# mayataka/robotoc

Hardware: NVIDIA H100
Metric: SQP-iterations/s (ANYmal N=40, batch=1024) at 1/2/4/8 H100 vs CPU ref (higher is better)
Workload: dtype f64

## Files before the change

### robotoc_b200/csrc/rbt_api.cu

```cuda
#include <cmath>
#include <cstdio>
#include <cstring>
#include <cstdint>
#include <cstdlib>
#include <string>
#include <utility>
#include <vector>

#include <cuda_runtime.h>
#include <dlfcn.h>

#include <algorithm>

#include "../../include/robotoc_b200.h"
#include "riccati_backward.cuh"
#include "riccati_forward.cuh"
#include "riccati_time_parallel.cuh"
#include "riccati_unconstr.cuh"
#include "stage_kernels.cuh"
#include "ustage_kernels.cuh"
#include "eval_kernels.cuh"
#include "line_search_kernels.cuh"
#include "rnea_kernels.cuh"
#include "contact_kernels.cuh"
// ... 88 lines not shown
  long long per;
  int scope;
  bool stage;
  Bindable* bind;
  int in;
};

long long buf_doubles(const BufDesc& d, bool stage_ready, int batch, int n_grid) {
  if (d.scope == SC_NONE || (d.stage && !stage_ready)) return -1;
  return d.per * batch * (d.scope == SC_GRID ? n_grid : 1);
}

struct Win {
  int b0, nb, n_grid;
  size_t rec() const { return size_t(b0) * n_grid; }
};

long long plan_bytes(const std::vector<Copy>& plan, bool up) {
  long long bytes = 0;
  for (const Copy& c : plan)
    if (c.up == up) bytes += (long long)(c.width * 8 * c.rows);
  return bytes;
}

}

struct rbt_handle {
  rbt_dims dims;
  rbt_layout L;
  int n_grid_max = 0, n_grid = 0, batch = 0, device = 0;
  double max_dts0 = 0.1;
  DevBuf<rbt_stage_ctrl> d_ctrl;
  std::vector<rbt_stage_ctrl> ctrl;
  Bindable d_kkt, d_ric, d_fact, d_dir, d_dx0;
  DevBuf<int> d_info;
  DevBuf<int> d_struct;
  int fxx_mode = RBT_FXX_AUTO;
  int tsegs = 0, n_sm = 0;
  DevBuf<double> d_tp_elem, d_tp_scan[2], d_tp_fmap, d_tp_dx;
  DevBuf<int> d_tp_fail;
  const double* tp_seeds = nullptr;
  bool kkt_from_condense = false;
  bool stage_ready = false;
  bool keep_info = false;
  rbt_stage_dims sdims;
  rbt_stage_layout S;
  rbt_constraint_table table;
  Bindable d_lin, d_con, d_ex, d_sol, d_xd;
  DevBuf<double> d_steps, d_ones;
  DevBuf<double> d_stage_perf, d_perf, d_x0in;
  DevBuf<int> d_tgt;
  DevBuf<double> d_limits;
  DevBuf<rbt::RneaModel> d_model;
  DevBuf<double> d_gains;
  DevBuf<double> d_cpos;
  bool cpos_set = false;
  int ls_trials = 0;
  DevBuf<double> d_ls_alphas, d_ls_trial, d_ls_stage_barrier, d_ls_barrier, d_ls_in, d_ls_filt, d_ls_step;
  DevBuf<int> d_ls_nfilt, d_ls_k;
  DevBuf<double> d_step_pack;
  long long launches = 0;
  DevBuf<double> d_wire;
  DevBuf<double> d_res_stage;
  DevBuf<double> d_sd_stage;
  DevBuf<rbt_wire_layout> d_W;
  long long w_ocp = 0;
// ... 37 lines not shown
  rbt_ulayout L;
  rbt_make_ulayout(nv, &L);
  return rbt_ulayout_field(&L, field);
}

int rbt_device_info(int device, int* sm, int* n_sm, char* name, int name_len) {
  cudaDeviceProp prop;
  if (cudaGetDeviceProperties(&prop, device) != cudaSuccess) {
    cudaGetLastError();
    return RBT_ERR_CUDA;
  }
  if (sm) *sm = prop.major * 10 + prop.minor;
  if (n_sm) *n_sm = prop.multiProcessorCount;
  if (name && name_len > 0) {
    std::strncpy(name, prop.name, name_len - 1);
    name[name_len - 1] = 0;
  }
  return RBT_OK;
}

int rbt_create(const rbt_dims* dims, int n_grid_max, int batch, int device, rbt_handle** out) {
  if (!dims || !out || n_grid_max < 2 || batch < 1 || dims->nv < 1 || dims->nu < 1 || dims->ns_max < 0) return RBT_ERR_ARG;
  if (dims->nv != CNV || dims->nu != CNU || dims->ns_max != CNS) return RBT_ERR_ARG;
  rbt_handle* h = new rbt_handle();
  h->dims = *dims;
  rbt_make_layout(dims, &h->L);
  h->n_grid_max = n_grid_max;
  h->batch = batch;
  h->device = device;
  *out = h;
  RBT_CUDA(h, cudaSetDevice(device));
  const size_t per = size_t(batch) * n_grid_max;
  RBT_CUDA(h, h->d_ctrl.ensure(size_t(n_grid_max)));
  RBT_CUDA(h, zeroed(h->d_kkt.own, per * h->L.k_stride));
  RBT_CUDA(h, zeroed(h->d_ric.own, per * h->L.r_stride));
  RBT_CUDA(h, zeroed(h->d_fact.own, per * h->L.f_stride));
  RBT_CUDA(h, zeroed(h->d_dir.own, per * h->L.d_stride));
  RBT_CUDA(h, h->d_dx0.own.ensure(size_t(batch) * h->L.nx));
  RBT_CUDA(h, zeroed(h->d_info, size_t(batch)));
  RBT_CUDA(h, zeroed(h->d_struct, 4));
  RBT_CUDA(h, cudaDeviceGetAttribute(&h->n_sm, cudaDevAttrMultiProcessorCount, device));
  return RBT_OK;
}

static int check_contacts(rbt_handle* h, const rbt_stage_dims& sd, const rbt_stage_ctrl* ctrl, int n_grid) {
  for (int i = 0; i < n_grid; ++i)
    if (ctrl[i].nf > sd.nf_max || ctrl[i].contact_mask >= (1 << sd.n_contacts)) {
      h->err = "[rbt_set_schedule] invalid argument: grid " + std::to_string(i) + " has more contacts than the stage layer was set up for";
      return RBT_ERR_ARG;
    }
  return RBT_OK;
}

int rbt_destroy(rbt_handle* h) {
  if (!h) return RBT_ERR_ARG;
  cudaSetDevice(h->device);
  delete h;
  return RBT_OK;
}

int rbt_set_schedule(rbt_handle* h, const rbt_stage_ctrl* ctrl, int n_grid, double max_dts0) {
  if (!h || !ctrl) return RBT_ERR_ARG;
  if (n_grid < 2 || n_grid > h->n_grid_max) {
    h->err = "[rbt_set_schedule] invalid argument: n_grid must be in [2, n_grid_max]";
    return RBT_ERR_ARG;
  }
  if (!(max_dts0 > 0)) {
    h->err = "[rbt_set_schedule] invalid argument: max_dts0 must be positive";
    return RBT_ERR_ARG;
  }
  for (int i = 0; i < n_grid; ++i) {
    const rbt_stage_ctrl& c = ctrl[i];
    const bool last = (i == n_grid - 1);
    if ((c.type == RBT_TERMINAL) != last || c.type < 0 || c.type > 3 || c.ns < 0 || c.ns > h->dims.ns_max ||
        (c.type == RBT_IMPACT && (i == 0 || last)) || (c.type == RBT_LIFT && i == 0)) {
      h->err = "[rbt_set_schedule] invalid argument: inconsistent stage control table at grid " + std::to_string(i);
      return RBT_ERR_ARG;
    }
    const int nf_max = 3 * RBT_MAX_CONTACTS;
    if (c.nf < 0 || c.nf > nf_max || c.nf % 3 != 0 || c.contact_mask < 0 || c.contact_mask >= (1 << RBT_MAX_CONTACTS) ||
        3 * __builtin_popcount((unsigned)c.contact_mask) != c.nf || c.ngrids_in_phase < 0 || !(c.dt >= 0.0) ||
        !(c.dt < 1.0e300) || (c.sto != 0 && c.sto != 1) || (c.sto_next != 0 && c.sto_next != 1) || c.ineq_gate < 0 ||
        c.ineq_gate > 2) {
      h->err = "[rbt_set_schedule] invalid argument: grid " + std::to_string(i) +
               ": need 0 <= nf <= 12, nf % 3 == 0, 3 * popcount(contact_mask) == nf, ngrids_in_phase >= 0, finite dt >= 0, "
               "ineq_gate in {0, 1, 2}";
      return RBT_ERR_ARG;
    }
    if (c.type == RBT_IMPACT && c.ns != 0) {
      h->err = "[rbt_set_schedule] invalid argument: an impact grid carries no switching constraint (grid " + std::to_string(i) + ")";
      return RBT_ERR_ARG;
    }
  }
  if (h->stage_ready && check_contacts(h, h->sdims, ctrl, n_grid) != RBT_OK) return RBT_ERR_ARG;
  RBT_CUDA(h, cudaSetDevice(h->device));
  RBT_CUDA(h, cudaMemcpy(h->d_ctrl.get(), ctrl, sizeof(rbt_stage_ctrl) * n_grid, cudaMemcpyHostToDevice));
  RBT_CUDA(h, cudaMemset(h->d_ric.get(), 0, size_t(h->batch) * n_grid * h->L.r_stride * 8));
  RBT_CUDA(h, cudaMemset(h->d_dir.get(), 0, size_t(h->batch) * n_grid * h->L.d_stride * 8));
  h->n_grid = n_grid;
  h->max_dts0 = max_dts0;
  h->ctrl.assign(ctrl, ctrl + n_grid);
  h->wire_dirty = true;
  return RBT_OK;
}

static BufDesc buf(rbt_handle* h, int which) {
  const rbt_layout& L = h->L;
  const rbt_stage_layout& S = h->S;
  const BufDesc t[] = {
       {h->d_kkt.get(), L.k_stride, SC_GRID, false, &h->d_kkt, IN_KKT},
       {h->d_ric.get(), L.r_stride, SC_GRID, false, &h->d_ric, -1},
       {h->d_fact.get(), L.f_stride, SC_GRID, false, &h->d_fact, -1},
       {h->d_dir.get(), L.d_stride, SC_GRID, false, &h->d_dir, -1},
       {h->d_dx0.get(), L.nx, SC_OCP, false, &h->d_dx0, IN_DX0},
       {nullptr, 0, SC_NONE, false, nullptr, -1},
       {h->d_lin.get(), S.l_stride, SC_GRID, true, &h->d_lin, IN_LIN},
       {h->d_con.get(), S.c_stride, SC_GRID, true, &h->d_con, IN_CON},
       {h->d_ex.get(), S.e_stride, SC_GRID, true, &h->d_ex, -1},
       {h->d_sol.get(), S.s_stride, SC_GRID, true, &h->d_sol, IN_SOL},
       {h->d_xd.get(), S.x_stride, SC_GRID, true, &h->d_xd, -1},
       {h->d_steps.get(), 2, SC_OCP, true, nullptr, -1},
       {h->d_perf.get(), 8, SC_OCP, true, nullptr, -1},
       {h->d_cpos.get(), 3 * S.ncon, SC_GRID, true, nullptr, IN_CPOS},
  };
  return which >= 0 && which < int(sizeof(t) / sizeof(t[0])) ? t[which] : BufDesc{nullptr, 0, SC_NONE, false, nullptr, -1};
}

long long rbt_buf_doubles(rbt_handle* h, int which) {
  return h ? buf_doubles(buf(h, which), h->stage_ready, h->batch, h->n_grid) : -1;
// ... 526 lines not shown
  rbt::StageParams p;
  const rbt_stage_layout& S = h->S;
  const size_t g0 = w.rec();
  p.K = h->L;
  p.S = S;
  p.tab = h->table;
  p.ctrl = h->d_ctrl.get();
  p.n_grid = h->n_grid;
  p.batch = w.nb;
  p.lin = h->d_lin.get() + g0 * S.l_stride;
  p.con = h->d_con.get() + g0 * S.c_stride;
  p.kkt = h->d_kkt.get() + g0 * h->L.k_stride;
  p.ex = h->d_ex.get() + g0 * S.e_stride;
  p.dir = h->d_dir.get() + g0 * h->L.d_stride;
  p.xd = h->d_xd.get() + g0 * S.x_stride;
  p.sol = h->d_sol.get() + g0 * S.s_stride;
  p.steps = h->d_steps.get() + 2 * size_t(w.b0);
  p.info = h->d_info.get() + w.b0;
  p.tgt = reinterpret_cast<const int4*>(h->d_tgt.get());
  p.row_level = h->d_tgt.get() + RBT_MAX_TARGETS * 4;
  return p;
}

#define RBT_STAGE_CHECK(h, what)                                  \
  if (!(h)) return RBT_ERR_ARG;                                   \
  if (!(h)->stage_ready || (h)->n_grid == 0) {                    \
    (h)->err = "[" what "] stage layer not set up / no schedule"; \
    return RBT_ERR_STATE;                                         \
  }                                                               \
  RBT_CUDA(h, cudaSetDevice((h)->device));

static int condense(rbt_handle* h, Win w, cudaStream_t st) {
  using C = rbt::CondCfg<CNV, CNU, CNS>;
  auto kern = rbt::condense_kernel<CNV, CNU, CNS>;
  if (!h->attr_cond) {
    RBT_CUDA(h, cudaFuncSetAttribute(kern, cudaFuncAttributeMaxDynamicSharedMemorySize, (int)C::SMEM_BYTES));
    h->attr_cond = true;
  }
  RBT_CUDA(h, cudaMemsetAsync(h->d_info.get() + w.b0, 0, size_t(w.nb) * sizeof(int), st));
  rbt::mjtjinv_kernel<CNV, CNU><<<(w.nb * h->n_grid + 1) / 2, 64, 0, st>>>(make_stage_params(h, w));
  RBT_CUDA(h, cudaGetLastError());
  if (h->ev_condense_mid) RBT_CUDA(h, cudaEventRecord(h->ev_condense_mid, st));
  kern<<<w.nb * h->n_grid, C::NTHREADS, C::SMEM_BYTES, st>>>(make_stage_params(h, w));
  RBT_CUDA(h, cudaGetLastError());
  h->launches += 2;
  h->keep_info = true;
  h->kkt_from_condense = true;
  return RBT_OK;
}

int rbt_condense(rbt_handle* h, void* stream) {
  RBT_STAGE_CHECK(h, "rbt_condense");
  return condense(h, full(h), (cudaStream_t)stream);
}

int rbt_set_condense_event(rbt_handle* h, void* cuda_event) {
  if (!h) return RBT_ERR_ARG;
  h->ev_condense_mid = (cudaEvent_t)cuda_event;
  return RBT_OK;
}

static int expand(rbt_handle* h, Win w, cudaStream_t st) {
  RBT_CUDA(h, cudaMemcpyAsync(h->d_steps.get() + 2 * size_t(w.b0), h->d_ones.get(), size_t(w.nb) * 2 * 8, cudaMemcpyDeviceToDevice, st));
  rbt::expand_kernel<CNV, CNU, CNS><<<w.nb * h->n_grid, rbt::XTHR, 0, st>>>(make_stage_params(h, w));
  RBT_CUDA(h, cudaGetLastError());
  h->launches += 1;
  return RBT_OK;
}

int rbt_expand_and_step_sizes(rbt_handle* h, void* stream) {
  RBT_STAGE_CHECK(h, "rbt_expand_and_step_sizes");
  return expand(h, full(h), (cudaStream_t)stream);
}

static int update(rbt_handle* h, Win w, cudaStream_t st) {
  rbt::update_kernel<CNV, CNU, CNS><<<w.nb * h->n_grid, rbt::XTHR, 0, st>>>(make_stage_params(h, w));
  RBT_CUDA(h, cudaGetLastError());
  h->launches += 1;
// ... 822 lines not shown
```

### robotoc_b200/csrc/stage_kernels.cuh

```cuda
#pragma once
#include "rbt_device.cuh"
#include "riccati_backward.cuh"
#include "../../include/rbt_stage_layout.h"

namespace rbt {

#define RBT_MAX_TARGETS 96
struct StageParams {
  rbt_layout K;
  rbt_stage_layout S;
  rbt_constraint_table tab;
  const rbt_stage_ctrl* ctrl;
  int n_grid;
  int batch;
  const double* lin;
  double* con;
  double* kkt;
  double* ex;
  double* dir;
  double* xd;
  double* sol;
  double* steps;
  int* info;
  const int4* tgt;
  const int* row_level;
};

__device__ __forceinline__ void cta_gemm(int ta, int tb, int m, int n, int k, double alpha, const double* A, int lda,
                                         const double* B, int ldb, double beta, double* C, int ldc) {
  for (int e = threadIdx.x; e < m * n; e += blockDim.x) {
    const int i = e % m, j = e / m;
    double acc = 0.0;
    for (int l = 0; l < k; ++l) {
      const double a = ta ? A[l + i * lda] : A[i + l * lda];
      const double b = tb ? B[j + l * ldb] : B[l + j * ldb];
      acc = fma(a, b, acc);
    }
    const double c0 = (beta == 0.0) ? 0.0 : beta * C[i + j * ldc];
    C[i + j * ldc] = fma(alpha, acc, c0);
  }
}

__device__ __forceinline__ void inv3_dev(const double* A, int lda, double* B, int ldb) {
  const double a = A[0], b = A[lda], c = A[2 * lda], d = A[1], e = A[1 + lda], f = A[1 + 2 * lda], g = A[2], h = A[2 + lda],
               i = A[2 + 2 * lda];
  const double det = a * (e * i - f * h) - b * (d * i - f * g) + c * (d * h - e * g);
  const double r = 1.0 / det;
  B[0] = (e * i - f * h) * r; B[ldb] = (c * h - b * i) * r; B[2 * ldb] = (b * f - c * e) * r;
  B[1] = (f * g - d * i) * r; B[1 + ldb] = (a * i - c * g) * r; B[1 + 2 * ldb] = (c * d - a * f) * r;
  B[2] = (d * h - e * g) * r; B[2 + ldb] = (b * g - a * h) * r; B[2 + 2 * ldb] = (a * e - b * d) * r;
}

__device__ __noinline__ void se3_jac_inverse_dev(const double* Jac, double* Jinv) {
  double tmp[9];
  for (int q = 0; q < 36; ++q) Jinv[q] = 0.0;
  inv3_dev(Jac, 6, Jinv, 6);
  inv3_dev(Jac + 3 + 18, 6, Jinv + 3 + 18, 6);
  for (int j = 0; j < 3; ++j)
// ... 194 lines not shown
template <int NV, int NU, int NFM>
struct CondCfg {
  static constexpr int NX = 2 * NV, NVF = NV + NFM;
  static constexpr int TX = num_tiles(NX), TF = num_tiles(NVF), TV = num_tiles(NV), TU = num_tiles(NU), TM = num_tiles(NFM);
  static constexpr int NWARPS = TX;
  static constexpr int NTHREADS = 32 * NWARPS;
  static constexpr int up2(int x) { return (x + 1) & ~1; }
  static constexpr int i_D = 0, i_IDC = i_D + up2(NVF * NX), i_Qaa = i_IDC + up2(NVF), i_Qff = i_Qaa + up2(NV),
                       i_Qqf = i_Qff + up2(NFM * NFM), IN1A = i_Qqf + up2(NV * NFM);
  static constexpr int i_Quu = IN1A, i_lx = i_Quu + up2(NU * NU), i_la = i_lx + up2(NX), i_lf = i_la + up2(NV),
                       i_lu = i_lf + up2(NFM), i_Fx = i_lu + up2(NU), i_lup = i_Fx + up2(NX), i_se3 = i_lup + 6,
                       IN1 = i_se3 + 108, IN1B = IN1 - IN1A;
  static constexpr int j_ha = 0, j_hf = j_ha + up2(NV), j_hx = j_hf + up2(NFM), j_hu = j_hx + up2(NX), j_fx = j_hu + up2(NU),
                       j_sc = j_fx + up2(NX), IN2 = j_sc + 4;
  static constexpr int o_in1 = 0;
  static constexpr int o_Z = o_in1 + IN1;
  static constexpr int o_R = o_Z + NVF * NVF;
  static constexpr int o_in2 = o_R + NVF * NX;
  static constexpr int o_vec = o_in2 + IN2;
  static constexpr int v_r = 0, v_laf = NVF, v_haf = 2 * NVF, v_Fi = 3 * NVF, v_FiS = v_Fi + 36, v_dQq = v_FiS + 36,
                       v_dQv = v_dQq + NV * NV, v_end = v_dQv + up2(NV);
  static constexpr int o_bar = (o_vec + v_end + 1) & ~1;
  static constexpr int SMEM_DOUBLES = o_bar + 2;
  static constexpr size_t SMEM_BYTES = size_t(SMEM_DOUBLES) * 8;
  static constexpr int QAF = 0, QUF = NFM * NX;
  static_assert(TF < NWARPS && TV <= NWARPS && 2 * TM < NWARPS, "one warp per row band, one warp left for the vectors");
  static_assert(NFM * NX + NFM * NV <= NVF * NX, "Qaf | Quf fit in the dIDCdqv buffer");
  static_assert((NFM * NX) % 2 == 0 && (NFM * NV) % 2 == 0, "Qaf | Quf are adjacent in the expansion record (one bulk store)");
};

#ifndef RBT_COND_MIN_CTAS
#define RBT_COND_MIN_CTAS 5
#endif
template <int NV, int NU, int NFM>
__global__ void __launch_bounds__(CondCfg<NV, NU, NFM>::NTHREADS, RBT_COND_MIN_CTAS) condense_kernel(const StageParams p) {
  using C = CondCfg<NV, NU, NFM>;
  constexpr int NX = C::NX, NVF = C::NVF, NTHR = C::NTHREADS, TX = C::TX, TF = C::TF, TV = C::TV, TU = C::TU, TM = C::TM;
  extern __shared__ __align__(16) double smem[];
  const rbt_layout& K = p.K;
  const rbt_stage_layout& S = p.S;
  const int tid = threadIdx.x, warp = tid >> 5, lane = tid & 31, g = lane >> 2, t = lane & 3;
  const size_t o = blockIdx.x;
  if (o >= size_t(p.batch) * p.n_grid) return;
  const int i = int(o % p.n_grid);
  const rbt_stage_ctrl c = p.ctrl[i];
  const double* lin = p.lin + o * S.l_stride;
  double* con = p.con + o * S.c_stride;
  double* kkt = p.kkt + o * K.k_stride;
  double* ex = p.ex + o * S.e_stride;
  constexpr int np = NV - NU;

  if (c.type == RBT_TERMINAL) {
    for (int e = tid; e < NX * NX; e += NTHR) kkt[K.k_Qxx + e] = lin[S.l_Qxx + e];
    for (int e = tid; e < NX; e += NTHR) kkt[K.k_lx + e] = lin[S.l_lx + e];
    if (np == 6 && tid == 0) se3_jac_inverse_dev(lin + S.l_se3 + 36, ex + S.e_Fqqpi);
    return;
  }
  const bool impact = (c.type == RBT_IMPACT);
  const bool pdipm = !impact || p.tab.impact_friction_cone != 0;
  const int nf = c.nf, nvf = NV + nf, ns = impact ? 0 : c.ns;
  const double dt = c.dt;
  double* in1 = smem + C::o_in1;
  double* sD = in1 + C::i_D;
  double* sQaf = sD + C::QAF;
  double* sQuf = sD + C::QUF;
  double* vIDC = in1 + C::i_IDC;
  double* vQaa = in1 + C::i_Qaa;
  double* sQff = in1 + C::i_Qff;
  double* sQqf = in1 + C::i_Qqf;
  const double* gQxx = lin + S.l_Qxx;
  double* gQuu = in1 + C::i_Quu;
  double* vlx = in1 + C::i_lx;
  double* vla = in1 + C::i_la;
  double* vlf = in1 + C::i_lf;
  double* vlu = in1 + C::i_lu;
  double* vFx = in1 + C::i_Fx;
  const double* vlup = in1 + C::i_lup;
  const double* sse3 = in1 + C::i_se3;
  double* sZ = smem + C::o_Z;
  double* sR = smem + C::o_R;
  const double* in2 = smem + C::o_in2;
  const double* vha = in2 + C::j_ha;
  const double* vhf = in2 + C::j_hf;
  const double* vhx = in2 + C::j_hx;
  const double* vhu = in2 + C::j_hu;
  const double* vfx = in2 + C::j_fx;
  const double* vsc = in2 + C::j_sc;
  double* vec = smem + C::o_vec;
  double* vr = vec + C::v_r;
  double* vlaf = vec + C::v_laf;
  double* vhaf = vec + C::v_haf;
  double* Fi = vec + C::v_Fi;
  double* FiS = vec + C::v_FiS;
  double* dQq = vec + C::v_dQq;
  double* dQv = vec + C::v_dQv;
  uint64_t* bar = reinterpret_cast<uint64_t*>(smem + C::o_bar);
  const int ncp = S.ncp, nbox = p.tab.n_box, ncon = p.tab.n_contacts, nc = S.nc;
  double* cSl = sR;
  double* sDq = sR + 3 * ncp;
  double* sDf = sDq + (S.l_dgdf - S.l_dgdq);
  const int gsz = (S.l_dgdf - S.l_dgdq) + ((15 * ncon + 1) & ~1);
  double* cW = sDq + ((gsz + 1) & ~1);
  double* cC = cW + ncp;

  if (tid == 0) {
    mbar_init(bar, 1);
    fence_mbar_init();
    uint32_t bytes = uint32_t(C::IN1 + NVF * NVF + C::IN2) * 8u;
    if (pdipm) bytes += uint32_t(3 * ncp + gsz) * 8u;
    mbar_expect_tx(bar, bytes);
    l2_prefetch_bulk(lin + S.l_Qxx, uint32_t(NX * NX) * 8u);
    tma_load_1d(in1, lin + S.l_D, uint32_t(C::IN1A) * 8u, bar);
    tma_load_1d(in1 + C::IN1A, lin + S.l_Quu, uint32_t(C::IN1B) * 8u, bar);
    tma_load_1d(sZ, ex + S.e_Z, uint32_t(NVF * NVF) * 8u, bar);
    tma_load_1d(smem + C::o_in2, lin + S.l_ha, uint32_t(C::IN2) * 8u, bar);
    if (pdipm) {
      tma_load_1d(cSl, con + S.c_slack, uint32_t(3 * ncp) * 8u, bar);
      tma_load_1d(sDq, lin + S.l_dgdq, uint32_t(gsz) * 8u, bar);
    }
  }
  __syncthreads();
  if (np == 6) {
    if (tid == 32 || tid == 33)
      se3_jac_inverse_dev(lin + S.l_se3 + (tid == 32 ? 36 : 72), tid == 32 ? ex + S.e_Fqqpi : Fi);
  }
  mbar_wait(bar, 0);

  if (nf < NFM) {
    for (int e = tid; e < NFM * NFM; e += NTHR)
      if ((e % NFM) >= nf || (e / NFM) >= nf) sQff[e] = 0.0;
    for (int e = nf * NV + tid; e < NV * NFM; e += NTHR) sQqf[e] = 0.0;
  }
  if (tid < NVF) {
    if (tid >= nvf) vIDC[tid] = 0.0;
    vhaf[tid] = impact ? 0.0 : (tid < NV ? vha[tid] : (tid - NV < nf ? -vhf[tid - NV] : 0.0));
    if (tid >= NV && tid - NV >= nf) vlf[tid - NV] = 0.0;
  }
  for (int e = tid; e < NV * NV + NV; e += NTHR) dQq[e] = 0.0;
  if (pdipm) {
    const double mu = p.tab.barrier;
    for (int r = tid; r < nc; r += NTHR) {
      const bool cone = r >= nbox;
      if (!cone && (impact || __ldg(p.row_level + r) + c.ineq_gate > 2)) {
        cW[r] = 0.0;
        cC[r] = 0.0;
        continue;
      }
// ... 14 lines not shown
      cC[r] = cd;
    }
    for (int ci = 0; ci < ncon; ++ci)
      if (!((c.contact_mask >> ci) & 1))
        for (int e = tid; e < 5 * NV + 15; e += NTHR) {
          if (e < 5 * NV) sDq[ci * 5 * NV + e] = 0.0;
          else sDf[ci * 15 + e - 5 * NV] = 0.0;
        }
  }
  __syncthreads();

  if (pdipm) {
    auto gather = [&](int tgt, double& w, double& gs) {
      const int4 e4 = __ldg(p.tgt + tgt);
      const int e[4] = {e4.x, e4.y, e4.z, e4.w};
      w = 0.0; gs = 0.0;
#pragma unroll
      for (int q = 0; q < 4; ++q)
        if (e[q] != 0) {
          const int r = (e[q] < 0 ? -e[q] : e[q]) - 1;
          w += cW[r];
          gs += (e[q] < 0) ? -cC[r] : cC[r];
        }
    };
    constexpr int KC = 5 * (NFM / 3);
    static_assert(KC % 4 == 0 && TV < NTHR / 32, "cone rows fill whole k-steps; at least one warp left for Qqf / Qff");
    if (warp < TV) {
      const int r0 = tile_off(warp, NV);
      double acc[TV][2];
#pragma unroll
      for (int n = 0; n < TV; ++n) acc[n][0] = acc[n][1] = 0.0;
#pragma unroll
      for (int ks = 0; ks < KC / 4; ++ks) {
        const int k = 4 * ks + t;
        const bool ok = k < 5 * ncon;
        const double* col = sDq + (k / 5) * 5 * NV + (k % 5);
        const double a = ok ? col[(r0 + g) * 5] * cW[nbox + k] : 0.0;
#pragma unroll
        for (int n = 0; n < TV; ++n) {
          const double bv = ok ? col[(tile_off(n, NV) + g) * 5] : 0.0;
          dmma884(acc[n][0], acc[n][1], a, bv);
        }
      }
#pragma unroll
      for (int n = 0; n < TV; ++n) {
        const int j0 = tile_off(n, NV);
        dQq[(r0 + g) + (j0 + 2 * t) * NV] = acc[n][0];
        dQq[(r0 + g) + (j0 + 2 * t + 1) * NV] = acc[n][1];
      }
      if (warp == 0 && lane < NV) {
        double a = 0.0;
        for (int ci = 0; ci < ncon; ++ci)
#pragma unroll
          for (int r = 0; r < 5; ++r) a = fma(sDq[ci * 5 * NV + r + lane * 5], cC[nbox + 5 * ci + r], a);
        vlx[lane] += a;
      } else if (warp == 1 && lane < 3 * ncon) {
        const int ci = lane / 3, j = lane % 3;
        if ((c.contact_mask >> ci) & 1) {
          const int fstack = 3 * __popc(c.contact_mask & ((1 << ci) - 1));
          double a = 0.0;
#pragma unroll
          for (int r = 0; r < 5; ++r) a = fma(sDf[ci * 15 + r + j * 5], cC[nbox + 5 * ci + r], a);
          vlf[fstack + j] += a;
        }
      }
    } else {
// ... 10 lines not shown
          const double* w5 = cW + nbox + 5 * ci;
          double acc = 0.0;
#pragma unroll
          for (int r = 0; r < 5; ++r) acc = fma(lhs[r] * w5[r], df[r], acc);
          if (isqf) sQqf[ii + (fstack + j) * NV] += acc;
          else sQff[(fstack + ii) + (fstack + j) * NFM] += acc;
        }
      }
    }
    __syncthreads();
    if (warp == 0 && lane < NV) {
      double w, gs;
      gather(lane, w, gs);
      vlx[lane] += gs;
      dQq[lane * (NV + 1)] += w;
    } else if (warp == 1 && lane < NV) {
      double w, gs;
      gather(NV + lane, w, gs);
      vlx[NV + lane] += gs;
      dQv[lane] = w;
    } else if (warp == 2 && lane < NV) {
      double w, gs;
      gather(2 * NV + lane, w, gs);
      vQaa[lane] += w;
      vla[lane] += gs;
    } else if (warp == 3 && lane < NU) {
      double w, gs;
      gather(3 * NV + lane, w, gs);
      gQuu[lane * (NU + 1)] += w;
      vlu[lane] += gs;
    }
    __syncthreads();
  }
  if (warp < TF) {
    const int i0 = tile_off(warp, NVF);
    double acc[TX][2];
#pragma unroll
    for (int n = 0; n < TX; ++n) acc[n][0] = acc[n][1] = 0.0;
    warp_mma_band<NVF, TX, NX>(
        acc, i0, [&](int ii, int k) { return sZ[ii + k * NVF]; }, [&](int k, int j) { return sD[k + j * NVF]; });
#pragma unroll
    for (int n = 0; n < TX; ++n) {
      const int j0 = tile_off(n, NX);
      sR[(i0 + g) + (j0 + 2 * t) * NVF] = acc[n][0];
      sR[(i0 + g) + (j0 + 2 * t + 1) * NVF] = acc[n][1];
    }
  } else {
    matvec_N4(sZ, NVF, NVF, NVF, vIDC, lane, 32, [&](int r, double a) { vr[r] = a; });
    if (np == 6)
      for (int e = lane; e < 36; e += 32) {
        const int ii = e % 6, j = e / 6;
        double acc = 0.0;
        for (int l = 0; l < 6; ++l) acc = fma(Fi[ii + l * 6], sse3[l + j * 6], acc);
        FiS[e] = acc;
      }
  }
  __syncthreads();

  if (warp < TM) {
    const int a0 = tile_off(warp, NFM);
    double acc[TX][2];
#pragma unroll
    for (int n = 0; n < TX; ++n) {
      const int j0 = tile_off(n, NX);
      acc[n][0] = (j0 + 2 * t < NV) ? -sQqf[(j0 + 2 * t) + (a0 + g) * NV] : 0.0;
      acc[n][1] = (j0 + 2 * t + 1 < NV) ? -sQqf[(j0 + 2 * t + 1) + (a0 + g) * NV] : 0.0;
    }
    warp_mma_band<NFM, TX, NX>(
        acc, a0, [&](int a, int l) { return -sQff[a + l * NFM]; }, [&](int l, int j) { return sR[(NV + l) + j * NVF]; });
#pragma unroll
    for (int n = 0; n < TX; ++n) {
      const int j0 = tile_off(n, NX);
      sQaf[(a0 + g) + (j0 + 2 * t) * NFM] = acc[n][0];
      sQaf[(a0 + g) + (j0 + 2 * t + 1) * NFM] = acc[n][1];
    }
  } else if (!impact && warp < 2 * TM) {
    const int a0 = tile_off(warp - TM, NFM);
    double acc[TV][2];
#pragma unroll
    for (int n = 0; n < TV; ++n) acc[n][0] = acc[n][1] = 0.0;
    warp_mma_band<NFM, TV, NV>(
        acc, a0, [&](int a, int l) { return sQff[a + l * NFM]; }, [&](int l, int j) { return sZ[(NV + l) + j * NVF]; });
#pragma unroll
    for (int n = 0; n < TV; ++n) {
      const int j0 = tile_off(n, NV);
      sQuf[(a0 + g) + (j0 + 2 * t) * NFM] = acc[n][0];
      sQuf[(a0 + g) + (j0 + 2 * t + 1) * NFM] = acc[n][1];
    }
  } else if (warp == NTHR / 32 - 1) {
    for (int r = lane; r < NVF; r += 32) {
      double v;
      if (r < NV) {
        v = vla[r] - vQaa[r] * vr[r];
      } else {
        double acc = 0.0;
        for (int l = 0; l < NFM; ++l) acc = fma(sQff[(r - NV) + l * NFM], vr[NV + l], acc);
        v = (r - NV < nf) ? -vlf[r - NV] - acc : 0.0;
      }
      vlaf[r] = v;
      ex[S.e_laf + r] = v;
      ex[S.e_r + r] = vr[r];
      if (!impact) ex[S.e_haf + r] = (c.sto || c.sto_next) ? vhaf[r] : 0.0;
      if (r < NV) ex[S.e_Qaa + r] = vQaa[r];
    }
  }
  __syncthreads();
  if (tid == 0) {
    tma_store_fence();
    tma_store_1d(ex + S.e_R, sR, uint32_t(NVF * NX) * 8u);
    tma_store_1d(ex + S.e_Qaf, sQaf, uint32_t(NFM * NX + NFM * NV) * 8u);
    tma_store_commit();
  }

  const int i0 = tile_off(warp, NX);
  {
    double acc[TX][2];
#pragma unroll
    for (int n = 0; n < TX; ++n) {
      const int j0 = tile_off(n, NX);
      const int r = i0 + g;
#pragma unroll
      for (int q = 0; q < 2; ++q) {
        const int cidx = j0 + 2 * t + q;
        double v = __ldg(gQxx + r + cidx * NX);
        if (r < NV && cidx < NV) v += dQq[r + cidx * NV];
        else if (r == cidx) v += dQv[r - NV];
        acc[n][q] = v;
      }
    }
    warp_mma_band<NV, TX, NX>(
        acc, i0, [&](int ii, int l) { return -sR[l + ii * NVF]; }, [&](int l, int j) { return -vQaa[l] * sR[l + j * NVF]; });
    warp_mma_band<NFM, TX, NX>(
        acc, i0, [&](int ii, int l) { return -sR[(NV + l) + ii * NVF]; }, [&](int l, int j) { return sQaf[l + j * NFM]; });
    warp_mma_band<NFM, TX, NX>(
        acc, i0, [&](int ii, int l) { return ii < NV ? sQqf[ii + l * NV] : 0.0; },
        [&](int l, int j) { return sR[(NV + l) + j * NVF]; });
    double* qxx_out = kkt + K.k_Qxx + (i0 + g) + 2 * t * NX;
#pragma unroll
    for (int n = 0; n < TX; ++n) {
      const int j0 = tile_off(n, NX);
      qxx_out[j0 * NX] = acc[n][0];
      qxx_out[(j0 + 1) * NX] = acc[n][1];
    }
  }
  if (!impact) {
    {
      double acc[TV][2];
#pragma unroll
      for (int n = 0; n < TV; ++n) acc[n][0] = acc[n][1] = 0.0;
      warp_mma_band<NV, TV, NV>(
          acc, i0, [&](int ii, int l) { return -sR[l + ii * NVF]; }, [&](int l, int j) { return vQaa[l] * sZ[l + j * NVF]; });
      warp_mma_band<NFM, TV, NV>(
          acc, i0, [&](int ii, int l) { return -sR[(NV + l) + ii * NVF]; }, [&](int l, int j) { return sQuf[l + j * NFM]; });
      warp_mma_band<NFM, TV, NV>(
          acc, i0, [&](int ii, int l) { return ii < NV ? -sQqf[ii + l * NV] : 0.0; },
          [&](int l, int j) { return sZ[(NV + l) + j * NVF]; });
      double* qxup_out = ex + S.e_Qxup + (i0 + g);
      double* qxu_out = kkt + K.k_Qxu + (i0 + g);
#pragma unroll
      for (int n = 0; n < TV; ++n) {
        const int j0 = tile_off(n, NV);
#pragma unroll
        for (int q = 0; q < 2; ++q) {
          const int j = j0 + 2 * t + q;
          double* dst = (j < np) ? qxup_out + j * NX : qxu_out + (j - np) * NX;
          *dst = acc[n][q];
        }
      }
    }
    if (warp < TV) {
      const int r0 = tile_off(warp, NV);
      double acc[TU][2];
#pragma unroll
      for (int n = 0; n < TU; ++n) {
        const int j0 = tile_off(n, NU);
        const int r = r0 + g;
        acc[n][0] = (r >= np) ? gQuu[(r - np) + (j0 + 2 * t) * NU] : 0.0;
        acc[n][1] = (r >= np) ? gQuu[(r - np) + (j0 + 2 * t + 1) * NU] : 0.0;
      }
      warp_mma_band<NV, TU, NU>(
          acc, r0, [&](int ii, int l) { return sZ[ii + l * NVF]; }, [&](int l, int j) { return vQaa[l] * sZ[l + (np + j) * NVF]; });
      warp_mma_band<NFM, TU, NU>(
          acc, r0, [&](int ii, int l) { return sZ[ii + (NV + l) * NVF]; }, [&](int l, int j) { return sQuf[l + (np + j) * NFM]; });
#pragma unroll
      for (int n = 0; n < TU; ++n) {
        const int j0 = tile_off(n, NU);
        const int r = r0 + g;
#pragma unroll
        for (int q = 0; q < 2; ++q) {
          if (r < np) ex[S.e_Quup + r + (j0 + 2 * t + q) * np] = acc[n][q];
          else kkt[K.k_Quu + (r - np) + (j0 + 2 * t + q) * NU] = acc[n][q];
        }
      }
    }
  }
  matvec_T(sR, NVF, NVF, NX, vlaf, tid, NTHR, [&](int ii, double a) {
    double v = vlx[ii] - a;
    if (ii < NV) {
      double a2 = 0.0;
      for (int l = 0; l < NFM; ++l) a2 = fma(sQqf[ii + l * NV], vr[NV + l], a2);
      v += a2;
    }
    kkt[K.k_lx + ii] = v;
  });
  if (!impact) {
    matvec_N4(sZ, NVF, NV, NVF, vlaf, tid, NTHR, [&](int ii, double a) {
      if (ii < np) ex[S.e_lup + ii] = vlup[ii] + a;
      else kkt[K.k_lu + ii - np] = vlu[ii - np] + a;
    });
  }
  const double sdt = impact ? 1.0 : dt;
  {
    constexpr int RP = NX / 2, CP = NTHR / RP;
    static_assert(NX % 2 == 0 && NV % 2 == 0 && NVF % 2 == 0 && CP >= 1, "row pairs never straddle the q | v boundary");
    if (tid < CP * RP) {
      const int r0 = 2 * (tid % RP), j0 = tid / RP;
      double* Fcol = kkt + K.k_Fxx + r0;
      if (r0 >= NV) {
        const double* rrow = sR + (r0 - NV);
#pragma unroll 2
        for (int j = j0; j < NX; j += CP) {
          const double2 rv = *reinterpret_cast<const double2*>(rrow + j * NVF);
          *reinterpret_cast<double2*>(Fcol + j * NX) =
              make_double2(fma(-sdt, rv.x, (j == r0) ? 1.0 : 0.0), fma(-sdt, rv.y, (j == r0 + 1) ? 1.0 : 0.0));
        }
      } else if (np == 6 && r0 < 6) {
#pragma unroll 2
        for (int j = j0; j < NX; j += CP) {
          double2 v = make_double2(0.0, 0.0);
          if (j < 6) v = make_double2(-FiS[r0 + j * 6], -FiS[r0 + 1 + j * 6]);
          else if (j >= NV && j < NV + 6 && !impact) v = make_double2(-dt * Fi[r0 + (j - NV) * 6], -dt * Fi[r0 + 1 + (j - NV) * 6]);
          *reinterpret_cast<double2*>(Fcol + j * NX) = v;
        }
      } else {
        const double dtv = impact ? 0.0 : dt;
#pragma unroll 2
        for (int j = j0; j < NX; j += CP)
          *reinterpret_cast<double2*>(Fcol + j * NX) = make_double2((j == r0) ? 1.0 : ((j == r0 + NV) ? dtv : 0.0),
                                                                    (j == r0 + 1) ? 1.0 : ((j == r0 + 1 + NV) ? dtv : 0.0));
// ... 18 lines not shown
    if (!impact) kkt[K.k_fx + ii] = f / c.ngrids_in_phase;
  }
  if (ns > 0) {
    const double* Phia = lin + S.l_Phia;
#pragma unroll 1
    for (int e = tid; e < ns * NV; e += NTHR) ex[S.e_Phia + e] = Phia[e];
#pragma unroll 1
    for (int e = tid; e < ns * NX; e += NTHR) {
      const int q = e % ns, j = e / ns;
      double acc = 0.0;
#pragma unroll 2
      for (int l = 0; l < NV; ++l) acc = fma(Phia[q + l * ns], sR[l + j * NVF], acc);
      kkt[K.k_Phix + e] = lin[S.l_Phix + e] - acc;
    }
#pragma unroll 1
    for (int e = tid; e < ns * NU; e += NTHR) {
      const int q = e % ns, j = e / ns;
      double acc = 0.0;
#pragma unroll 2
      for (int l = 0; l < NV; ++l) acc = fma(Phia[q + l * ns], sZ[l + (np + j) * NVF], acc);
      kkt[K.k_Phiu + e] = acc;
    }
#pragma unroll 1
    for (int q = tid; q < ns; q += NTHR) {
      double acc = 0.0;
#pragma unroll 2
      for (int l = 0; l < NV; ++l) acc = fma(Phia[q + l * ns], vr[l], acc);
      kkt[K.k_p + q] = lin[S.l_p + q] - acc;
      kkt[K.k_Phit + q] = (lin[S.l_Phit + q] - acc) / c.ngrids_in_phase;
    }
  }
  if (!impact && (c.sto || c.sto_next)) {
    const double g1 = 1.0 / c.ngrids_in_phase;
    matvec_T(sR, NVF, NVF, NX, vhaf, tid, NTHR, [&](int ii, double a) {
      double v = vhx[ii] - a;
      if (ii < NV) {
        double a2 = 0.0;
        for (int l = 0; l < NFM; ++l) a2 = fma(sQqf[ii + l * NV], vr[NV + l], a2);
        v += a2 / dt;
      }
      kkt[K.k_hx + ii] = v * g1;
    });
    for (int ii = tid; ii < NU; ii += NTHR) {
      double acc = 0.0;
#pragma unroll 1
      for (int l = 0; l < NVF; ++l) acc = fma(sZ[(np + ii) + l * NVF], vhaf[l], acc);
      kkt[K.k_hu + ii] = (vhu[ii] + acc) * g1;
    }
    if (tid == NTHR - 1) {
      double h = vsc[0];
      for (int l = 0; l < NVF; ++l) h = fma(-vr[l], vhaf[l], h);
      const double Qtt = vsc[1] * g1 * g1;
      kkt[K.k_sc + 0] = Qtt;
      kkt[K.k_sc + 1] = -Qtt;
      kkt[K.k_sc + 2] = h * g1;
      kkt[K.k_sc + 3] = 0.0;
    }
  }
  if (tid == 0) tma_store_wait_read();
}

struct WireParams {
  const rbt_wire_layout* W;
  int n_grid, l_stride;
  long long ocp_stride;
  const double* wire;
  double* lin;
  const double* res;
  double* con;
  int c_stride, c_res, ncp;
};

__global__ void __launch_bounds__(128) unpack_wire_kernel(const WireParams p) {
  const int i = int(blockIdx.x % p.n_grid);
  const size_t b = blockIdx.x / p.n_grid;
  const rbt_wire_layout& W = p.W[i];
  const double* wire = p.wire + b * size_t(p.ocp_stride) + W.ocp_off;
  double* lin = p.lin + size_t(blockIdx.x) * p.l_stride;
  const int nseg = W.nseg;
  for (int k = 0; k < W.nzero; ++k)
    for (int e = threadIdx.x; e < W.zero[k].n; e += 128) lin[W.zero[k].lin_off + e] = 0.0;
  __syncthreads();
  for (int k = 0; k < nseg; ++k) {
    const rbt_wire_seg g = W.seg[k];
// ... 416 lines not shown
```

Measured before the change: 218,000.

## Specialize condense kernel on active contact count and skip inactive contact blocks

Grid stages are split on the host into two classes, those with at most six active contact forces and the rest, using an index list. A separate condense_kernel instantiation is launched for each class, and the small-contact variant restricts the Z load, the band MMAs and the matvecs to NV+6 columns while zero-filling the unused rows of R and Qaf. A contact-mask check also skips k-slices of one GEMM for inactive contacts. This cuts FLOPs and shared-memory traffic for stages with few contacts, at the cost of an extra kernel launch and indirect stage indexing. Correctness depends on active forces always occupying the leading columns.

Measured after the change: 219,600, median of 6. About the same (+0.7%).

```diff
diff --git a/robotoc_b200/csrc/rbt_api.cu b/robotoc_b200/csrc/rbt_api.cu
--- a/robotoc_b200/csrc/rbt_api.cu
+++ b/robotoc_b200/csrc/rbt_api.cu
@@ -144,6 +144,8 @@
   double max_dts0 = 0.1;
   DevBuf<rbt_stage_ctrl> d_ctrl;
   std::vector<rbt_stage_ctrl> ctrl;
+  DevBuf<int> d_cls;
+  int n_cls[2] = {0, 0};
   Bindable d_kkt, d_ric, d_fact, d_dir, d_dx0;
   DevBuf<int> d_info;
   DevBuf<int> d_struct;
@@ -247,6 +249,7 @@
   RBT_CUDA(h, cudaSetDevice(device));
   const size_t per = size_t(batch) * n_grid_max;
   RBT_CUDA(h, h->d_ctrl.ensure(size_t(n_grid_max)));
+  RBT_CUDA(h, h->d_cls.ensure(size_t(n_grid_max)));
   RBT_CUDA(h, zeroed(h->d_kkt.own, per * h->L.k_stride));
   RBT_CUDA(h, zeroed(h->d_ric.own, per * h->L.r_stride));
   RBT_CUDA(h, zeroed(h->d_fact.own, per * h->L.f_stride));
@@ -310,6 +313,13 @@
   if (h->stage_ready && check_contacts(h, h->sdims, ctrl, n_grid) != RBT_OK) return RBT_ERR_ARG;
   RBT_CUDA(h, cudaSetDevice(h->device));
   RBT_CUDA(h, cudaMemcpy(h->d_ctrl.get(), ctrl, sizeof(rbt_stage_ctrl) * n_grid, cudaMemcpyHostToDevice));
+  std::vector<int> cls[2];
+  for (int i = 0; i < n_grid; ++i)
+    cls[(RBT_COND_ACTIVE_NF && ctrl[i].type != RBT_TERMINAL && ctrl[i].nf <= 6) ? 0 : 1].push_back(i);
+  cls[0].insert(cls[0].end(), cls[1].begin(), cls[1].end());
+  RBT_CUDA(h, cudaMemcpy(h->d_cls.get(), cls[0].data(), sizeof(int) * n_grid, cudaMemcpyHostToDevice));
+  h->n_cls[0] = n_grid - int(cls[1].size());
+  h->n_cls[1] = int(cls[1].size());
   RBT_CUDA(h, cudaMemset(h->d_ric.get(), 0, size_t(h->batch) * n_grid * h->L.r_stride * 8));
   RBT_CUDA(h, cudaMemset(h->d_dir.get(), 0, size_t(h->batch) * n_grid * h->L.d_stride * 8));
   h->n_grid = n_grid;
@@ -902,18 +912,25 @@
 
 static int condense(rbt_handle* h, Win w, cudaStream_t st) {
   using C = rbt::CondCfg<CNV, CNU, CNS>;
-  auto kern = rbt::condense_kernel<CNV, CNU, CNS>;
+  void (*const kern[2])(rbt::StageParams) = {rbt::condense_kernel<CNV, CNU, CNS, 6>, rbt::condense_kernel<CNV, CNU, CNS, CNS>};
   if (!h->attr_cond) {
-    RBT_CUDA(h, cudaFuncSetAttribute(kern, cudaFuncAttributeMaxDynamicSharedMemorySize, (int)C::SMEM_BYTES));
+    for (auto k : kern) RBT_CUDA(h, cudaFuncSetAttribute(k, cudaFuncAttributeMaxDynamicSharedMemorySize, (int)C::SMEM_BYTES));
     h->attr_cond = true;
   }
   RBT_CUDA(h, cudaMemsetAsync(h->d_info.get() + w.b0, 0, size_t(w.nb) * sizeof(int), st));
-  rbt::mjtjinv_kernel<CNV, CNU><<<(w.nb * h->n_grid + 1) / 2, 64, 0, st>>>(make_stage_params(h, w));
-  RBT_CUDA(h, cudaGetLastError());
+  rbt::StageParams p = make_stage_params(h, w);
+  rbt::mjtjinv_kernel<CNV, CNU><<<(w.nb * h->n_grid + 1) / 2, 64, 0, st>>>(p);
+  RBT_CUDA(h, cudaGetLastError());
+  h->launches += 1;
   if (h->ev_condense_mid) RBT_CUDA(h, cudaEventRecord(h->ev_condense_mid, st));
-  kern<<<w.nb * h->n_grid, C::NTHREADS, C::SMEM_BYTES, st>>>(make_stage_params(h, w));
-  RBT_CUDA(h, cudaGetLastError());
-  h->launches += 2;
+  for (int k = 0, off = 0; k < 2; off += h->n_cls[k++]) {
+    if (h->n_cls[k] == 0) continue;
+    p.sel = h->d_cls.get() + off;
+    p.n_sel = h->n_cls[k];
+    kern[k]<<<w.nb * p.n_sel, C::NTHREADS, C::SMEM_BYTES, st>>>(p);
+    RBT_CUDA(h, cudaGetLastError());
+    h->launches += 1;
+  }
   h->keep_info = true;
   h->kkt_from_condense = true;
   return RBT_OK;
diff --git a/robotoc_b200/csrc/stage_kernels.cuh b/robotoc_b200/csrc/stage_kernels.cuh
--- a/robotoc_b200/csrc/stage_kernels.cuh
+++ b/robotoc_b200/csrc/stage_kernels.cuh
@@ -6,6 +6,9 @@
 namespace rbt {
 
 #define RBT_MAX_TARGETS 96
+#ifndef RBT_COND_ACTIVE_NF
+#define RBT_COND_ACTIVE_NF 1
+#endif
 struct StageParams {
   rbt_layout K;
   rbt_stage_layout S;
@@ -24,6 +27,8 @@
   int* info;
   const int4* tgt;
   const int* row_level;
+  const int* sel = nullptr;
+  int n_sel = 0;
 };
 
 __device__ __forceinline__ void cta_gemm(int ta, int tb, int m, int n, int k, double alpha, const double* A, int lda,
@@ -284,17 +289,21 @@
 #ifndef RBT_COND_MIN_CTAS
 #define RBT_COND_MIN_CTAS 5
 #endif
-template <int NV, int NU, int NFM>
+template <int NV, int NU, int NFM, int NFA>
 __global__ void __launch_bounds__(CondCfg<NV, NU, NFM>::NTHREADS, RBT_COND_MIN_CTAS) condense_kernel(const StageParams p) {
   using C = CondCfg<NV, NU, NFM>;
-  constexpr int NX = C::NX, NVF = C::NVF, NTHR = C::NTHREADS, TX = C::TX, TF = C::TF, TV = C::TV, TU = C::TU, TM = C::TM;
+  constexpr int NX = C::NX, NVF = C::NVF, NTHR = C::NTHREADS, TX = C::TX, TV = C::TV, TU = C::TU;
+  constexpr int NVA = NV + NFA, TFA = num_tiles(NVA), TMA = num_tiles(NFA);
+  constexpr int MROWS = NFA < 8 ? 8 : NFA;
+  static_assert(NFA <= NFM && NFA % 3 == 0 && TFA < C::NWARPS && 2 * TMA < C::NWARPS, "one warp per band, one for the vectors");
+  static_assert((NVF * NVA) % 2 == 0, "the leading NVA columns of Z are a whole number of 16-byte units");
   extern __shared__ __align__(16) double smem[];
   const rbt_layout& K = p.K;
   const rbt_stage_layout& S = p.S;
   const int tid = threadIdx.x, warp = tid >> 5, lane = tid & 31, g = lane >> 2, t = lane & 3;
-  const size_t o = blockIdx.x;
-  if (o >= size_t(p.batch) * p.n_grid) return;
-  const int i = int(o % p.n_grid);
+  if (blockIdx.x >= unsigned(p.batch) * unsigned(p.n_sel)) return;
+  const int i = __ldg(p.sel + blockIdx.x % unsigned(p.n_sel));
+  const size_t o = size_t(blockIdx.x / unsigned(p.n_sel)) * p.n_grid + i;
   const rbt_stage_ctrl c = p.ctrl[i];
   const double* lin = p.lin + o * S.l_stride;
   double* con = p.con + o * S.c_stride;
@@ -358,13 +367,13 @@
   if (tid == 0) {
     mbar_init(bar, 1);
     fence_mbar_init();
-    uint32_t bytes = uint32_t(C::IN1 + NVF * NVF + C::IN2) * 8u;
+    uint32_t bytes = uint32_t(C::IN1 + NVF * NVA + C::IN2) * 8u;
     if (pdipm) bytes += uint32_t(3 * ncp + gsz) * 8u;
     mbar_expect_tx(bar, bytes);
     l2_prefetch_bulk(lin + S.l_Qxx, uint32_t(NX * NX) * 8u);
     tma_load_1d(in1, lin + S.l_D, uint32_t(C::IN1A) * 8u, bar);
     tma_load_1d(in1 + C::IN1A, lin + S.l_Quu, uint32_t(C::IN1B) * 8u, bar);
-    tma_load_1d(sZ, ex + S.e_Z, uint32_t(NVF * NVF) * 8u, bar);
+    tma_load_1d(sZ, ex + S.e_Z, uint32_t(NVF * NVA) * 8u, bar);
     tma_load_1d(smem + C::o_in2, lin + S.l_ha, uint32_t(C::IN2) * 8u, bar);
     if (pdipm) {
       tma_load_1d(cSl, con + S.c_slack, uint32_t(3 * ncp) * 8u, bar);
@@ -445,6 +454,8 @@
       for (int n = 0; n < TV; ++n) acc[n][0] = acc[n][1] = 0.0;
 #pragma unroll
       for (int ks = 0; ks < KC / 4; ++ks) {
+        if (RBT_COND_ACTIVE_NF && !((c.contact_mask >> ((4 * ks) / 5)) & 1) && !((c.contact_mask >> ((4 * ks + 3) / 5)) & 1))
+          continue;
         const int k = 4 * ks + t;
         const bool ok = k < 5 * ncon;
         const double* col = sDq + (k / 5) * 5 * NV + (k % 5);
@@ -521,12 +532,12 @@
     }
     __syncthreads();
   }
-  if (warp < TF) {
-    const int i0 = tile_off(warp, NVF);
+  if (warp < TFA) {
+    const int i0 = tile_off(warp, NVA);
     double acc[TX][2];
 #pragma unroll
     for (int n = 0; n < TX; ++n) acc[n][0] = acc[n][1] = 0.0;
-    warp_mma_band<NVF, TX, NX>(
+    warp_mma_band<NVA, TX, NX>(
         acc, i0, [&](int ii, int k) { return sZ[ii + k * NVF]; }, [&](int k, int j) { return sD[k + j * NVF]; });
 #pragma unroll
     for (int n = 0; n < TX; ++n) {
@@ -534,8 +545,8 @@
       sR[(i0 + g) + (j0 + 2 * t) * NVF] = acc[n][0];
       sR[(i0 + g) + (j0 + 2 * t + 1) * NVF] = acc[n][1];
     }
-  } else {
-    matvec_N4(sZ, NVF, NVF, NVF, vIDC, lane, 32, [&](int r, double a) { vr[r] = a; });
+  } else if (warp == TFA) {
+    matvec_N4(sZ, NVF, NVF, NVA, vIDC, lane, 32, [&](int r, double a) { vr[r] = a; });
     if (np == 6)
       for (int e = lane; e < 36; e += 32) {
         const int ii = e % 6, j = e / 6;
@@ -543,11 +554,14 @@
         for (int l = 0; l < 6; ++l) acc = fma(Fi[ii + l * 6], sse3[l + j * 6], acc);
         FiS[e] = acc;
       }
+  } else if constexpr (NVA < NVF) {
+    for (int e = tid - 32 * (TFA + 1); e < (NVF - NVA) * NX; e += NTHR - 32 * (TFA + 1))
+      sR[NVA + e % (NVF - NVA) + (e / (NVF - NVA)) * NVF] = 0.0;
   }
   __syncthreads();
 
-  if (warp < TM) {
-    const int a0 = tile_off(warp, NFM);
+  if (warp < TMA) {
+    const int a0 = tile_off(warp, NFA);
     double acc[TX][2];
 #pragma unroll
     for (int n = 0; n < TX; ++n) {
@@ -555,7 +569,7 @@
       acc[n][0] = (j0 + 2 * t < NV) ? -sQqf[(j0 + 2 * t) + (a0 + g) * NV] : 0.0;
       acc[n][1] = (j0 + 2 * t + 1 < NV) ? -sQqf[(j0 + 2 * t + 1) + (a0 + g) * NV] : 0.0;
     }
-    warp_mma_band<NFM, TX, NX>(
+    warp_mma_band<NFA, TX, NX>(
         acc, a0, [&](int a, int l) { return -sQff[a + l * NFM]; }, [&](int l, int j) { return sR[(NV + l) + j * NVF]; });
 #pragma unroll
     for (int n = 0; n < TX; ++n) {
@@ -563,12 +577,12 @@
       sQaf[(a0 + g) + (j0 + 2 * t) * NFM] = acc[n][0];
       sQaf[(a0 + g) + (j0 + 2 * t + 1) * NFM] = acc[n][1];
     }
-  } else if (!impact && warp < 2 * TM) {
-    const int a0 = tile_off(warp - TM, NFM);
+  } else if (!impact && warp < 2 * TMA) {
+    const int a0 = tile_off(warp - TMA, NFA);
     double acc[TV][2];
 #pragma unroll
     for (int n = 0; n < TV; ++n) acc[n][0] = acc[n][1] = 0.0;
-    warp_mma_band<NFM, TV, NV>(
+    warp_mma_band<NFA, TV, NV>(
         acc, a0, [&](int a, int l) { return sQff[a + l * NFM]; }, [&](int l, int j) { return sZ[(NV + l) + j * NVF]; });
 #pragma unroll
     for (int n = 0; n < TV; ++n) {
@@ -583,7 +597,7 @@
         v = vla[r] - vQaa[r] * vr[r];
       } else {
         double acc = 0.0;
-        for (int l = 0; l < NFM; ++l) acc = fma(sQff[(r - NV) + l * NFM], vr[NV + l], acc);
+        for (int l = 0; l < NFA; ++l) acc = fma(sQff[(r - NV) + l * NFM], vr[NV + l], acc);
         v = (r - NV < nf) ? -vlf[r - NV] - acc : 0.0;
       }
       vlaf[r] = v;
@@ -592,6 +606,11 @@
       if (!impact) ex[S.e_haf + r] = (c.sto || c.sto_next) ? vhaf[r] : 0.0;
       if (r < NV) ex[S.e_Qaa + r] = vQaa[r];
     }
+  } else if constexpr (MROWS < NFM) {
+    constexpr int NZ = NFM - MROWS, FREE = NTHR - 64 * TMA - 32;
+    if (warp >= 2 * TMA)
+      for (int e = tid - 64 * TMA; e < NZ * (impact ? NX : NX + NV); e += FREE)
+        sQaf[MROWS + e % NZ + (e / NZ) * NFM] = 0.0;
   }
   __syncthreads();
   if (tid == 0) {
@@ -619,9 +638,9 @@
     }
     warp_mma_band<NV, TX, NX>(
         acc, i0, [&](int ii, int l) { return -sR[l + ii * NVF]; }, [&](int l, int j) { return -vQaa[l] * sR[l + j * NVF]; });
-    warp_mma_band<NFM, TX, NX>(
+    warp_mma_band<NFA, TX, NX>(
         acc, i0, [&](int ii, int l) { return -sR[(NV + l) + ii * NVF]; }, [&](int l, int j) { return sQaf[l + j * NFM]; });
-    warp_mma_band<NFM, TX, NX>(
+    warp_mma_band<NFA, TX, NX>(
         acc, i0, [&](int ii, int l) { return ii < NV ? sQqf[ii + l * NV] : 0.0; },
         [&](int l, int j) { return sR[(NV + l) + j * NVF]; });
     double* qxx_out = kkt + K.k_Qxx + (i0 + g) + 2 * t * NX;
@@ -639,9 +658,9 @@
       for (int n = 0; n < TV; ++n) acc[n][0] = acc[n][1] = 0.0;
       warp_mma_band<NV, TV, NV>(
           acc, i0, [&](int ii, int l) { return -sR[l + ii * NVF]; }, [&](int l, int j) { return vQaa[l] * sZ[l + j * NVF]; });
-      warp_mma_band<NFM, TV, NV>(
+      warp_mma_band<NFA, TV, NV>(
           acc, i0, [&](int ii, int l) { return -sR[(NV + l) + ii * NVF]; }, [&](int l, int j) { return sQuf[l + j * NFM]; });
-      warp_mma_band<NFM, TV, NV>(
+      warp_mma_band<NFA, TV, NV>(
           acc, i0, [&](int ii, int l) { return ii < NV ? -sQqf[ii + l * NV] : 0.0; },
           [&](int l, int j) { return sZ[(NV + l) + j * NVF]; });
       double* qxup_out = ex + S.e_Qxup + (i0 + g);
@@ -669,7 +688,7 @@
       }
       warp_mma_band<NV, TU, NU>(
           acc, r0, [&](int ii, int l) { return sZ[ii + l * NVF]; }, [&](int l, int j) { return vQaa[l] * sZ[l + (np + j) * NVF]; });
-      warp_mma_band<NFM, TU, NU>(
+      warp_mma_band<NFA, TU, NU>(
           acc, r0, [&](int ii, int l) { return sZ[ii + (NV + l) * NVF]; }, [&](int l, int j) { return sQuf[l + (np + j) * NFM]; });
 #pragma unroll
       for (int n = 0; n < TU; ++n) {
@@ -683,17 +702,17 @@
       }
     }
   }
-  matvec_T(sR, NVF, NVF, NX, vlaf, tid, NTHR, [&](int ii, double a) {
+  matvec_T(sR, NVF, NVA, NX, vlaf, tid, NTHR, [&](int ii, double a) {
     double v = vlx[ii] - a;
     if (ii < NV) {
       double a2 = 0.0;
-      for (int l = 0; l < NFM; ++l) a2 = fma(sQqf[ii + l * NV], vr[NV + l], a2);
+      for (int l = 0; l < NFA; ++l) a2 = fma(sQqf[ii + l * NV], vr[NV + l], a2);
       v += a2;
     }
     kkt[K.k_lx + ii] = v;
   });
   if (!impact) {
-    matvec_N4(sZ, NVF, NV, NVF, vlaf, tid, NTHR, [&](int ii, double a) {
+    matvec_N4(sZ, NVF, NV, NVA, vlaf, tid, NTHR, [&](int ii, double a) {
       if (ii < np) ex[S.e_lup + ii] = vlup[ii] + a;
       else kkt[K.k_lu + ii - np] = vlu[ii - np] + a;
     });
@@ -778,11 +797,11 @@
   }
   if (!impact && (c.sto || c.sto_next)) {
     const double g1 = 1.0 / c.ngrids_in_phase;
-    matvec_T(sR, NVF, NVF, NX, vhaf, tid, NTHR, [&](int ii, double a) {
+    matvec_T(sR, NVF, NVA, NX, vhaf, tid, NTHR, [&](int ii, double a) {
       double v = vhx[ii] - a;
       if (ii < NV) {
         double a2 = 0.0;
-        for (int l = 0; l < NFM; ++l) a2 = fma(sQqf[ii + l * NV], vr[NV + l], a2);
+        for (int l = 0; l < NFA; ++l) a2 = fma(sQqf[ii + l * NV], vr[NV + l], a2);
         v += a2 / dt;
       }
       kkt[K.k_hx + ii] = v * g1;
@@ -790,12 +809,12 @@
     for (int ii = tid; ii < NU; ii += NTHR) {
       double acc = 0.0;
 #pragma unroll 1
-      for (int l = 0; l < NVF; ++l) acc = fma(sZ[(np + ii) + l * NVF], vhaf[l], acc);
+      for (int l = 0; l < NVA; ++l) acc = fma(sZ[(np + ii) + l * NVF], vhaf[l], acc);
       kkt[K.k_hu + ii] = (vhu[ii] + acc) * g1;
     }
     if (tid == NTHR - 1) {
       double h = vsc[0];
-      for (int l = 0; l < NVF; ++l) h = fma(-vr[l], vhaf[l], h);
+      for (int l = 0; l < NVA; ++l) h = fma(-vr[l], vhaf[l], h);
       const double Qtt = vsc[1] * g1 * g1;
       kkt[K.k_sc + 0] = Qtt;
       kkt[K.k_sc + 1] = -Qtt;
```
